# trinhvg/MoMA

Measured on AMD Instinct MI355X. Metric: images/sec MoMA train step (EffNet-B0 224px, K=65536), higher is better.
Workload: dtype bf16

## Files before the change

include/moma_hip.h:

```cpp
#ifndef MOMA_HIP_H
#define MOMA_HIP_H

#include <stddef.h>
#include <stdint.h>

#ifdef __cplusplus
extern "C" {
#endif

#define MOMA_ABI_VERSION 4

enum { MOMA_PREC_F32 = 0, MOMA_PREC_BF16 = 1 };
enum { MOMA_DT_F32 = 0, MOMA_DT_BF16 = 1 };

enum {
    MOMA_OK = 0,
    MOMA_E_NULL = -1,
    MOMA_E_SHAPE = -2,
    MOMA_E_DTYPE = -3,
    MOMA_E_ALIGN = -4,
    MOMA_E_WORKSPACE = -5,
    MOMA_E_UNSUPPORTED = -6
};

// ... 127 lines not shown
    const void* x;
    const void* pack;
    const float* b_qkv;
    const float* b_proj;
    float* y;
    void* qkv16;
    void* attn16;
    float* lse;
    void* qpack;
    float qpack_scale;
    int x_dtype;
} moma_mha_module_t;
size_t moma_mha_pack_bytes(int d);
int moma_mha_pack_weights(const float* w_qkv, const float* w_proj, void* pack, int d, int with_transposed,
                          moma_stream_t stream);
int moma_mha_fwd_fast(const moma_mha_module_t* modules, int n_modules, int N, int d, int H, moma_stream_t stream);
size_t moma_mha_bwd_fast_workspace_bytes(int N, int d, int H);
int moma_mha_bwd_fast(const void* pack, const void* x, int x_dtype, const void* qkv16, const void* attn16, const float* lse,
                      const float* dy, float* dx, float* dw_qkv, float* db_qkv, float* dw_proj, float* db_proj,
                      void* workspace, size_t workspace_bytes, int N, int d, int H, moma_stream_t stream);

enum { MOMA_ACT_NONE = 0, MOMA_ACT_SILU = 1, MOMA_ACT_RELU = 2 };
size_t moma_bn_workspace_bytes(int C);
int moma_bn_fwd(const void* x, void* out, const float* gamma, const float* beta, float* running_mean,
                float* running_var, float* save_mean, float* save_invstd, void* workspace,
                size_t workspace_bytes, int N, int C, int HW, int dtype, int act, int training,
                float momentum, float eps, void* plane_mean, moma_stream_t stream);
int moma_bn_bwd(const void* x, const void* dout, const float* gamma, const float* beta,
                const float* save_mean, const float* save_invstd, void* dx, float* dgamma, float* dbeta,
                void* workspace, size_t workspace_bytes, int N, int C, int HW, int dtype, int act,
                int training, const void* dplane_mean, moma_stream_t stream);
int moma_bn_prepare(const void* x, const float* gamma, const float* beta, float* running_mean,
                    float* running_var, float* save_mean, float* save_invstd, float* scale_shift,
                    void* workspace, size_t workspace_bytes, int N, int C, int HW, int dtype, int training,
                    float momentum, float eps, moma_stream_t stream);

size_t moma_dwconv_workspace_bytes(int C, int K);
int moma_dwconv_fwd(const void* x, const float* w, void* y, int N, int C, int H, int W, int OH, int OW,
                    int K, int stride, int pad_top, int pad_left, int dtype, moma_stream_t stream);
int moma_dwconv_bwd_data(const void* dy, const float* w, void* dx, int N, int C, int H, int W, int OH,
                         int OW, int K, int stride, int pad_top, int pad_left, int dtype,
                         moma_stream_t stream);
int moma_dwconv_bwd_weight(const void* x, const void* dy, float* dw, void* workspace,
                           size_t workspace_bytes, int N, int C, int H, int W, int OH, int OW, int K,
                           int stride, int pad_top, int pad_left, int dtype, moma_stream_t stream);
int moma_dwconv_fwd_pre(const void* x, const float* w, void* y, int N, int C, int H, int W, int OH, int OW,
                        int K, int stride, int pad_top, int pad_left, int dtype, const float* scale_shift,
                        int act, moma_stream_t stream);
int moma_dwconv_bwd_weight_pre(const void* x, const void* dy, float* dw, void* workspace,
                               size_t workspace_bytes, int N, int C, int H, int W, int OH, int OW, int K,
                               int stride, int pad_top, int pad_left, int dtype, const float* scale_shift,
                               int act, moma_stream_t stream);

int moma_plane_mean(const void* x, void* mean, int NC, int HW, int dtype, moma_stream_t stream);
int moma_se_gate_fwd(const void* x, const void* s, void* out, int NC, int HW, int dtype, moma_stream_t stream);
int moma_se_gate_bwd(const void* x, const void* s, const void* dout, void* dx, void* ds, int NC, int HW,
                     int dtype, moma_stream_t stream);

#ifdef __cplusplus
}
#endif
#endif
```

moma_amd/_lib.py:

```python
from __future__ import annotations

import ctypes as C
import os

_HERE = os.path.dirname(os.path.abspath(__file__))
LIB_PATH = os.environ.get("MOMA_HIP_LIB", os.path.join(_HERE, "lib", "libmoma_hip.so"))

PREC_F32, PREC_BF16 = 0, 1
DT_F32, DT_BF16 = 0, 1
LAYOUT_NCHW, LAYOUT_NHWC = 0, 1
NST_MAX_C, NST_ROW_BLOCK = 256, 32
RKD_MAX_B = 1024
SP_MAX_B = 1024
PKT_MAX_B = 1024
MHA_SAVE_PROBS, MHA_SAVE_LSE = 0, 1
ABI_VERSION = 4
EMA_BLOCK_ELEMS = 4096

_p = C.c_void_p
_i = C.c_int
_l = C.c_int64
_f = C.c_float
_z = C.c_size_t

# ... 6 lines not shown
    "moma_enqueue_mirror": (_i, [_p, _p, _p, _i, _l, _i, _i, _p]),
    "moma_queue_prefetch": (_i, [_p, _z, _p]),
    "moma_infonce_logits": (_i, [_p, _p, _p, _p, _i, _i, _i, _f, _i, _i, _p]),
    "moma_infonce_logits_bwd": (_i, [_p, _p, _p, _p, _i, _i, _i, _f, _i, _i, _p]),
    "moma_infonce_logits_bwd_workspace_bytes": (_z, [_i, _i, _i]),
    "moma_infonce_logits_bwd_ws": (_i, [_p, _p, _p, _p, _i, _i, _i, _f, _i, _i, _p, _z, _p]),
    "moma_infonce_logits_bwd_kq": (_i, [_p, _p, _p, _p, _i, _i, _i, _f, _i, _p]),
    "moma_infonce_fused_workspace_bytes": (_z, [_i, _i, _i, _i, _i]),
    "moma_infonce_fused": (_i, [_p, _p, _p, _i, _i, _i, _f, _p, _p, _p, _p, _p, _z, _i, _i, _p]),
    "moma_infonce_fused_ex": (_i, [_p, _p, _p, _i, _i, _i, _f, _p, _p, _p, _p, _p, _z, _i, _i, _p, _p, _p]),
    "moma_infonce_qpack_bytes": (_z, [_i, _i]),
    "moma_infonce_fused_q": (_i, [_p, _p, _p, _p, _i, _i, _i, _f, _p, _p, _p, _p, _p, _z, _i, _i, _p, _p, _p, _p]),
    "moma_infonce_fused_enqueue": (_i, [_p, _p, _p, _p, _i, _i, _i, _f, _p, _p, _p, _p, _p, _z, _i, _i, _p, _i, _l, _p, _p, _p, _p, _p]),
    "moma_infonce_fused_multi_workspace_bytes": (_z, [_i, _i, _i, _i, _i, _i]),
    "moma_infonce_fused_multi": (_i, [_p, _i, _i, _i, _i, _f, _p, _z, _i, _i, _p]),
    "moma_crd_workspace_bytes": (_z, [_i, _i, _i]),
    "moma_crd_fused": (_i, [_p, _p, _p, _p, _p, _i, _i, _i, _l, _f, _p, _i, _p, _p, _p, _p, _p, _z, _p]),
    "moma_crd_scores": (_i, [_p, _p, _p, _p, _p, _i, _i, _i, _l, _f, _p, _i, _p, _p, _p, _p, _z, _p]),
    "moma_crd_scores_bwd": (_i, [_p, _p, _p, _p, _p, _p, _p, _i, _i, _i, _l, _f, _p, _p, _p, _p, _z, _p]),
    "moma_crd_update": (_i, [_p, _p, _p, _p, _p, _i, _i, _l, _f, _p, _p]),
    "moma_at_workspace_bytes": (_z, [_i] * 8),
    "moma_at_map": (_i, [_p, _p] + [_i] * 8 + [_p, _z, _p]),
    "moma_at_pair": (_i, [_p, _p, _i, _i, _p, _p, _p, _p, _p, _p, _p, _p]),
    "moma_at_bwd": (_i, [_p, _p, _p, _p] + [_i] * 8 + [_p]),
    "moma_nst_workspace_bytes": (_z, [_i] * 3),
    "moma_nst_gram": (_i, [_p, _p] + [_i] * 8 + [_p, _z, _p, _p, _p, _p, _p, _p]),
    "moma_nst_bwd": (_i, [_p, _p, _p, _z, _p, _p, _p, _p] + [_i] * 8 + [_p]),
    "moma_rkd_workspace_bytes": (_z, [_i]),
    "moma_rkd_dist": (_i, [_p, _i, _i, _i, _p, _p]),
    "moma_rkd_terms": (_i, [_p, _p, _i, _f, _f, _p, _z, _p, _p, _p, _p]),
    "moma_rkd_bwd": (_i, [_p, _p, _p, _p, _i, _i, _i, _p]),
    "moma_sp_workspace_bytes": (_z, [_i, _l]),
    "moma_sp_gram": (_i, [_p, _i, _l, _i, _p, _z, _p]),
    "moma_sp_terms": (_i, [_p, _z, _l, _p, _z, _l, _i, _p, _p, _p, _p, _p, _p]),
    "moma_sp_bwd": (_i, [_p, _p, _p, _p, _i, _l, _i, _p]),
    "moma_pkt_workspace_bytes": (_z, [_i]),
    "moma_pkt_gram": (_i, [_p, _i, _i, _i, _p, _p]),
    "moma_pkt_gram_pair": (_i, [_p, _i, _i, _p, _i, _i, _i, _p, _p, _p]),
    "moma_pkt_terms":(_i, [_p, _p, _i, _p, _z, _p, _p, _p]),
    "moma_pkt_bwd": (_i, [_p, _p, _p, _p, _i, _i, _i, _p]),
    "moma_mha_fwd": (_i,[_p, _p, _p, _p, _p, _p, _p, _p, _p, _i, _i, _i, _i, _p]),
    "moma_mha_saved_state": (_i, [_i, _i, _i, _i]),
    "moma_mha_pack_bytes": (_z, [_i]),
    "moma_mha_pack_weights": (_i, [_p, _p, _p, _i, _i, _p]),
    "moma_mha_fwd_fast": (_i, [_p, _i, _i, _i, _i, _p]),
    "moma_mha_bwd_fast_workspace_bytes": (_z, [_i, _i, _i]),
    "moma_mha_bwd_fast": (_i, [_p, _p, _i, _p, _p, _p, _p, _p, _p, _p, _p, _p, _p, _z, _i, _i, _i, _p]),
    "moma_dwconv_workspace_bytes": (_z, [_i, _i]),
    "moma_dwconv_fwd": (_i, [_p, _p, _p] + [_i] * 11 + [_p]),
    "moma_dwconv_bwd_data": (_i, [_p, _p, _p] + [_i] * 11 + [_p]),
    "moma_dwconv_bwd_weight": (_i, [_p, _p, _p, _p, _z] + [_i] * 11 + [_p]),
    "moma_dwconv_fwd_pre": (_i, [_p, _p, _p] + [_i] * 11 + [_p, _i, _p]),
    "moma_dwconv_bwd_weight_pre": (_i, [_p, _p, _p, _p, _z] + [_i] * 11 + [_p, _i, _p]),
    "moma_plane_mean": (_i, [_p, _p, _i, _i, _i, _p]),
    "moma_se_gate_fwd": (_i, [_p, _p, _p, _i, _i, _i, _p]),
    "moma_se_gate_bwd": (_i, [_p, _p, _p, _p, _p, _i, _i, _i, _p]),
    "moma_bn_workspace_bytes": (_z, [_i]),
    "moma_bn_fwd": (_i, [_p, _p, _p, _p, _p, _p, _p, _p, _p, _z, _i, _i, _i, _i, _i, _i, _f, _f, _p, _p]),
    "moma_bn_bwd": (_i, [_p, _p, _p, _p, _p, _p, _p, _p, _p, _p, _z, _i, _i, _i, _i, _i, _i, _p, _p]),
    "moma_bn_prepare": (_i, [_p, _p, _p, _p, _p, _p, _p, _p, _p, _z, _i, _i, _i, _i, _i, _f, _f, _p]),
    "moma_mha_bwd_workspace_bytes": (_z, [_i, _i, _i, _i]),
    "moma_mha_bwd": (_i, [_p, _p, _p, _p, _p, _p, _p, _p, _p, _p, _p, _p, _p, _z, _i, _i, _i, _i, _p]),
}



class InfoNCETerm(C.Structure):
    _fields_ = [("q", _p), ("k", _p), ("queue", _p), ("loss_rows", _p), ("lse", _p), ("top1", _p), ("dq", _p)]


class MhaModule(C.Structure):
    _fields_ = [("x", _p), ("pack", _p), ("b_qkv", _p), ("b_proj", _p), ("y", _p), ("qkv16", _p), ("attn16", _p),
                ("lse", _p), ("qpack", _p), ("qpack_scale", _f), ("x_dtype", _i)]


_lib = None


class MomaHipError(RuntimeError):
    pass


def load():
    global _lib
    if _lib is not None:
        return _lib
    import torch
    if not os.path.exists(LIB_PATH):
        raise MomaHipError(
            f"libmoma_hip.so not found at {LIB_PATH}: build it with `python -m moma_amd.build` "
            "(hipcc --offload-arch=gfx950). There is no CPU fallback for the MoMA hot path.")
    lib = C.CDLL(LIB_PATH)
    for name, (res, args) in SIGNATURES.items():
        try:
            fn = getattr(lib, name)
        except AttributeError as e:
            raise MomaHipError(f"{LIB_PATH} does not export {name}") from e
        fn.restype = res
        fn.argtypes = args
    v = lib.moma_version()
    if v != ABI_VERSION:
        raise MomaHipError(f"libmoma_hip ABI version {v} != binding version {ABI_VERSION}; rebuild")
    _lib = lib
    return lib


# ... 5 lines not shown
```

moma_amd/backbones/efficientnet.py:

```python
import math
import os

import torch
import torch.nn as nn
import torch.nn.functional as F

_DW_MODE = os.environ.get("MOMA_DW", "hip")
_BN_MODE = os.environ.get("MOMA_BN", "hip")
_SE_MODE = os.environ.get("MOMA_SE", "hip")
_BNDW_FUSE = os.environ.get("MOMA_BNDW", "1")

_B0_STAGES = [
    (1, 3, 1, 1, 32, 16, 0.25),
    (2, 3, 2, 6, 16, 24, 0.25),
    (2, 5, 2, 6, 24, 40, 0.25),
    (3, 3, 2, 6, 40, 80, 0.25),
    (3, 5, 1, 6, 80, 112, 0.25),
    (4, 5, 2, 6, 112, 192, 0.25),
    (1, 3, 1, 6, 192, 320, 0.25),
]
_BN_MOM, _BN_EPS = 0.01, 1e-3


class _DepthwiseNative(torch.autograd.Function):

    @staticmethod
    def forward(ctx, x, w, stride, padding, groups):
        w = w.to(x.dtype)
        with torch.backends.cudnn.flags(enabled=False):
            y = F.conv2d(x, w, None, stride, padding, 1, groups)
        ctx.save_for_backward(x, w)
        ctx.cfg = (stride, padding, groups)
        return y

    @staticmethod
    def backward(ctx, gy):
        x, w = ctx.saved_tensors
        stride, padding, groups = ctx.cfg
        pad = padding if isinstance(padding, (tuple, list)) else (padding, padding)
        with torch.backends.cudnn.flags(enabled=False):
            gx, gw, _ = torch.ops.aten.convolution_backward(
                gy.contiguous(), x, w, None, list(stride), list(pad), [1, 1], False, [0, 0], groups,
                [ctx.needs_input_grad[0], ctx.needs_input_grad[1], False])
        return gx, (gw.float() if gw is not None else None), None, None, None


class _CachedCast(torch.autograd.Function):

    @staticmethod
    def forward(ctx, master, cached):
        ctx.dtype = master.dtype
        return cached.view_as(cached)

    @staticmethod
    def backward(ctx, g):
        return g.to(ctx.dtype), None


_WCACHE = os.environ.get("MOMA_WCACHE", "1") == "1"


def _same_pad(ih, iw, kh, kw, sh, sw):
    return (max((math.ceil(ih / sh) - 1) * sh + kh - ih, 0), max((math.ceil(iw / sw) - 1) * sw + kw - iw, 0))


class SamePadConv2d(nn.Conv2d):

    def __init__(self, cin, cout, kernel_size, stride=1, groups=1, bias=True):
        super().__init__(cin, cout, kernel_size, stride=stride, padding=0, groups=groups, bias=bias)
        self._wc = self._bc = None
        self._wc_live = False

    def _params(self, x):
        if self._wc_live and x.is_cuda and x.dtype == torch.bfloat16:
            track = torch.is_grad_enabled()
            w = _CachedCast.apply(self.weight, self._wc) if (track and self.weight.requires_grad) else self._wc
            b = None
            if self.bias is not None:
                b = _CachedCast.apply(self.bias, self._bc) if (track and self.bias.requires_grad) else self._bc
            return w, b
        return self.weight, self.bias

    def _is_depthwise(self):
        return self.groups > 1 and self.groups == self.in_channels == self.out_channels and self.bias is None

    def forward(self, x):
        ih, iw = x.shape[-2:]
        kh, kw = self.kernel_size
        sh, sw = self.stride
        ph, pw = _same_pad(ih, iw, kh, kw, sh, sw)
        depthwise = self._is_depthwise()
        if depthwise and x.is_cuda and _DW_MODE == "hip" and kh == kw and sh == sw and self.dilation == (1, 1):
            from .. import ops
            if ops.dwconv_supported(kh, sh):
                if torch.is_autocast_enabled():
                    x = x.to(torch.get_autocast_dtype("cuda"))
                if x.dtype in (torch.float32, torch.bfloat16):
                    return ops.dwconv(x, self.weight, sh, ph // 2, pw // 2, math.ceil(ih / sh), math.ceil(iw / sw))
        pad = (ph // 2, pw // 2)
        if ph % 2 or pw % 2:
            x = F.pad(x, [pw // 2, pw - pw // 2, ph // 2, ph - ph // 2])
            pad = 0
        if depthwise and x.is_cuda and _DW_MODE in ("hip", "aten"):
            if torch.is_autocast_enabled():
                x = x.to(torch.get_autocast_dtype("cuda"))
            return _DepthwiseNative.apply(x, self.weight, self.stride, pad, self.groups)
        if self._wc_live and torch.is_autocast_enabled() and x.is_cuda and x.dtype != torch.bfloat16 and \
                torch.get_autocast_dtype("cuda") == torch.bfloat16:
            x = x.to(torch.bfloat16)
        w, b = self._params(x)
        return F.conv2d(x, w, b, self.stride, pad, self.dilation, self.groups)


class BatchNorm2d(nn.BatchNorm2d):

    _nbt_pending = 0

    def _flush_nbt(self):
        if self._nbt_pending and self.num_batches_tracked is not None:
            self.num_batches_tracked.add_(self._nbt_pending)
        self._nbt_pending = 0

    def _save_to_state_dict(self, destination, prefix, keep_vars):
        self._flush_nbt()
        super()._save_to_state_dict(destination, prefix, keep_vars)

    def _load_from_state_dict(self, *args, **kwargs):
        self._nbt_pending = 0
        super()._load_from_state_dict(*args, **kwargs)

    def forward(self, x, act=None, want_mean=False):
        if _BN_MODE == "hip" and x.is_cuda and x.dtype in (torch.float32, torch.bfloat16) and self.momentum is not None:
            from .. import ops
            use_batch = self.training or self.running_mean is None
            if self.training and self.track_running_stats and self.num_batches_tracked is not None:
                self._nbt_pending += 1
            return ops.bn_act(x, self.weight, self.bias, self.running_mean, self.running_var, use_batch,
                              self.momentum, self.eps, act, want_mean)
        if _BN_MODE == "aten" and x.is_cuda:
            with torch.backends.cudnn.flags(enabled=False):
                y = super().forward(x)
        else:
            y = super().forward(x)
        y = F.silu(y) if act == "silu" else (F.relu(y) if act == "relu" else y)
        return (y, F.adaptive_avg_pool2d(y, 1)) if want_mean else y


def _drop_connect(x, p, training):
    if not training or not p:
        return x
    keep = 1.0 - p
    mask = torch.floor(keep + torch.rand([x.shape[0], 1, 1, 1], dtype=x.dtype, device=x.device))
    return x / keep * mask


class MBConvBlock(nn.Module):
    def __init__(self, kernel, stride, expand, cin, cout, se_ratio):
        super().__init__()
        mid = cin * expand
        self.expand, self.stride, self.cin, self.cout = expand, stride, cin, cout
        if expand != 1:
            self._expand_conv = SamePadConv2d(cin, mid, 1, bias=False)
            self._bn0 = BatchNorm2d(mid, momentum=_BN_MOM, eps=_BN_EPS)
# ... 134 lines not shown
```

moma_amd/csrc/api.hip:

```cpp
#include "common.hpp"

using namespace moma;

namespace {
inline int hip_rc(hipError_t e) { return e == hipSuccess ? MOMA_OK : (int)e; }
inline bool bad_prec(int p) { return p != MOMA_PREC_F32 && p != MOMA_PREC_BF16; }
inline bool bad_dt(int t) { return t != MOMA_DT_F32 && t != MOMA_DT_BF16; }
inline bool misaligned(const void* p, size_t a) { return ((uintptr_t)p % a) != 0; }
inline size_t align_up(size_t x, size_t a) { return (x + a - 1) / a * a; }

#define MOMA_TRY(expr)                         \
    do {                                       \
        hipError_t _e = (expr);                \
        if (_e != hipSuccess) return (int)_e;  \
    } while (0)

GemmArgs gemm(const float* A, const void* B, float* C, int M, int N, int K, long lda, long ldb, long ldc, int tA,
              int tB, float alpha, int prec) {
    GemmArgs g{};
    g.A = A; g.B = B; g.C = C; g.bias = nullptr;
    g.M = M; g.N = N; g.K = K; g.lda = lda; g.ldb = ldb; g.ldc = ldc;
    g.strideA = g.strideB = g.strideC = 0; g.batch = 1;
    g.transA = tA; g.transB = tB; g.alpha = alpha; g.splitk = 1; g.atomic = 0; g.splitC = 0;
    g.b_dtype = MOMA_DT_F32; g.prec = prec;
// ... 471 lines not shown

int moma_dwconv_fwd(const void* x, const float* w, void* y, int N, int C, int H, int W, int OH, int OW, int K, int stride,
                    int pad_top, int pad_left, int dtype, moma_stream_t stream) {
    if (!x || !w || !y) return MOMA_E_NULL;
    const int rc = dw_check(N, C, H, W, OH, OW, K, stride, pad_top, pad_left, dtype);
    if (rc != MOMA_OK) return rc;
    return hip_rc(launch_dw_fwd(x, w, y, N, C, H, W, OH, OW, K, stride, pad_top, pad_left, dtype, nullptr, MOMA_ACT_NONE,
                                (hipStream_t)stream));
}

static bool bad_act(int act) { return act != MOMA_ACT_NONE && act != MOMA_ACT_SILU && act != MOMA_ACT_RELU; }

int moma_dwconv_fwd_pre(const void* x, const float* w, void* y, int N, int C, int H, int W, int OH, int OW, int K, int stride,
                        int pad_top, int pad_left, int dtype, const float* scale_shift, int act, moma_stream_t stream) {
    if (!x || !w || !y || !scale_shift) return MOMA_E_NULL;
    const int rc = dw_check(N, C, H, W, OH, OW, K, stride, pad_top, pad_left, dtype);
    if (rc != MOMA_OK) return rc;
    if (bad_act(act)) return MOMA_E_DTYPE;
    return hip_rc(launch_dw_fwd(x, w, y, N, C, H, W, OH, OW, K, stride, pad_top, pad_left, dtype, scale_shift, act,
                                (hipStream_t)stream));
}

int moma_dwconv_bwd_data(const void* dy, const float* w, void* dx, int N, int C, int H, int W, int OH, int OW, int K,
                         int stride, int pad_top, int pad_left, int dtype, moma_stream_t stream) {
    if (!dy || !w || !dx) return MOMA_E_NULL;
    const int rc = dw_check(N, C, H, W, OH, OW, K, stride, pad_top, pad_left, dtype);
    if (rc != MOMA_OK) return rc;
    return hip_rc(launch_dw_bwd_data(dy, w, dx, N, C, H, W, OH, OW, K, stride, pad_top, pad_left, dtype, (hipStream_t)stream));
}

int moma_dwconv_bwd_weight(const void* x, const void* dy, float* dw, void* workspace, size_t workspace_bytes, int N, int C,
                           int H, int W, int OH, int OW, int K, int stride, int pad_top, int pad_left, int dtype,
                           moma_stream_t stream) {
    if (!x || !dy || !dw || !workspace) return MOMA_E_NULL;
    const int rc = dw_check(N, C, H, W, OH, OW, K, stride, pad_top, pad_left, dtype);
    if (rc != MOMA_OK) return rc;
    if (workspace_bytes < moma_dwconv_workspace_bytes(C, K)) return MOMA_E_WORKSPACE;
    return hip_rc(launch_dw_bwd_weight(x, dy, dw, (float*)workspace, workspace_bytes / sizeof(float), N, C, H, W, OH, OW, K,
                                       stride, pad_top, pad_left, dtype, nullptr, MOMA_ACT_NONE, (hipStream_t)stream));
}

int moma_dwconv_bwd_weight_pre(const void* x, const void* dy, float* dw, void* workspace, size_t workspace_bytes, int N, int C,
                               int H, int W, int OH, int OW, int K, int stride, int pad_top, int pad_left, int dtype,
                               const float* scale_shift, int act, moma_stream_t stream) {
    if (!x || !dy || !dw || !workspace || !scale_shift) return MOMA_E_NULL;
    const int rc = dw_check(N, C, H, W, OH, OW, K, stride, pad_top, pad_left, dtype);
    if (rc != MOMA_OK) return rc;
    if (bad_act(act)) return MOMA_E_DTYPE;
    if (workspace_bytes < moma_dwconv_workspace_bytes(C, K)) return MOMA_E_WORKSPACE;
    return hip_rc(launch_dw_bwd_weight(x, dy, dw, (float*)workspace, workspace_bytes / sizeof(float), N, C, H, W, OH, OW, K,
                                       stride, pad_top, pad_left, dtype, scale_shift, act, (hipStream_t)stream));
}

static int se_check(int NC, int HW, int dtype) {
    if (NC <= 0 || HW <= 0) return MOMA_E_SHAPE;
    if (dtype != MOMA_DT_F32 && dtype != MOMA_DT_BF16) return MOMA_E_DTYPE;
    return MOMA_OK;
}
int moma_plane_mean(const void* x, void* mean, int NC, int HW, int dtype, moma_stream_t stream) {
    if (!x || !mean) return MOMA_E_NULL;
    const int rc = se_check(NC, HW, dtype);
    return rc != MOMA_OK ? rc : hip_rc(launch_plane_mean(x, mean, NC, HW, dtype, (hipStream_t)stream));
}
int moma_se_gate_fwd(const void* x, const void* s, void* out, int NC, int HW, int dtype, moma_stream_t stream) {
    if (!x || !s || !out) return MOMA_E_NULL;
    const int rc = se_check(NC, HW, dtype);
    return rc != MOMA_OK ? rc : hip_rc(launch_se_gate_fwd(x, s, out, NC, HW, dtype, (hipStream_t)stream));
}
int moma_se_gate_bwd(const void* x, const void* s, const void* dout, void* dx, void* ds, int NC, int HW, int dtype,
                     moma_stream_t stream) {
    if (!x || !s || !dout || !dx || !ds) return MOMA_E_NULL;
    const int rc = se_check(NC, HW, dtype);
    return rc != MOMA_OK ? rc : hip_rc(launch_se_gate_bwd(x, s, dout, dx, ds, NC, HW, dtype, (hipStream_t)stream));
}

static int crd_check(int B, int d, int K1, int64_t n_data, float T) {
    if (B <= 0 || d < 4 || d % 4 != 0 || K1 < 2 || n_data <= 0 || !(T > 0.f)) return MOMA_E_SHAPE;
    if (d > 2048 || B > 65535) return MOMA_E_UNSUPPORTED;
    return MOMA_OK;
}
static bool crd_misaligned(const void* a, const void* b, const void* c, const void* d, const void* e = nullptr,
                           const void* f = nullptr, const void* g = nullptr, const void* h = nullptr) {
    return misaligned(a, 16) || misaligned(b, 16) || misaligned(c, 16) || misaligned(d, 16) || misaligned(e, 16) ||
           misaligned(f, 16) || misaligned(g, 16) || misaligned(h, 16);
}

size_t moma_crd_workspace_bytes(int B, int d, int K1) {
    if (crd_check(B, d, K1, 1, 1.f) != MOMA_OK) return 0;
    return crd_workspace_bytes(B, d, K1);
}

int moma_crd_fused(const float* v1, const float* v2, const float* memory_v1, const float* memory_v2, const int64_t* idx,
                   int B, int d, int K1, int64_t n_data, float T, float* Z, int set_z, float* loss, float* dv1, float* dv2,
                   int32_t* bad_index, void* workspace, size_t workspace_bytes, moma_stream_t stream) {
    if (!v1 || !v2 || !memory_v1 || !memory_v2 || !idx || !Z || !loss || !bad_index || !workspace) return MOMA_E_NULL;
    if ((dv1 == nullptr) != (dv2 == nullptr)) return MOMA_E_NULL;
    const int rc = crd_check(B, d, K1, n_data, T);
    if (rc != MOMA_OK) return rc;
    if (crd_misaligned(v1, v2, memory_v1, memory_v2, dv1, dv2, workspace) || misaligned(idx, 8) || misaligned(Z, 4) ||
        misaligned(loss, 4) || misaligned(bad_index, 4))
        return MOMA_E_ALIGN;
    if (workspace_bytes < crd_workspace_bytes(B, d, K1)) return MOMA_E_WORKSPACE;
    return hip_rc(launch_crd_fused(v1, v2, memory_v1, memory_v2, idx, B, d, K1, n_data, T, Z, set_z, loss, dv1, dv2, bad_index,
                                   workspace, (hipStream_t)stream));
}

// ... 272 lines not shown
```

moma_amd/csrc/common.hpp:

```cpp
#pragma once
#include <hip/hip_runtime.h>
#include <stdint.h>
#include <initializer_list>
#include <type_traits>
#include "../../include/moma_hip.h"

namespace moma {

typedef __attribute__((ext_vector_type(8))) __bf16 bf16x8;
typedef __attribute__((ext_vector_type(4))) __bf16 bf16x4;
typedef __attribute__((ext_vector_type(4))) float f32x4;
typedef __attribute__((ext_vector_type(16))) float f32x16;
typedef unsigned short bf16_raw;

constexpr int WAVE = 64;

__device__ __forceinline__ float bf16_to_f32(bf16_raw v) {
    return __uint_as_float(((unsigned)v) << 16);
}
__device__ __forceinline__ bf16_raw f32_to_bf16(float f) {
    __bf16 b = (__bf16)f;
    return *reinterpret_cast<bf16_raw*>(&b);
}

// ... 242 lines not shown
    void* queue16;
    float* queue32;
    const float* rows;
    int n;
    int64_t index;
    int K, d;
};
hipError_t launch_infonce_flash(const float* q, const float* k, const void* queue, int B, int d, int K, float inv_T,
                                float* loss_rows, float* lse, int32_t* top1, float* dq, void* ws, int qdtype,
                                hipStream_t st, hipEvent_t ev_begin = nullptr, hipEvent_t ev_end = nullptr,
                                const void* q_packed = nullptr, hipEvent_t ev_call_end = nullptr,
                                const EnqueueJob* enq = nullptr);
size_t infonce_qpack_bytes(int B, int d);
bool infonce_multi_supported(int n_terms, int B, int d, int K, int qdtype, int prec);
size_t infonce_multi_workspace_bytes(int n_terms, int B, int d, int K);
hipError_t launch_infonce_multi(const moma_infonce_term_t* terms, int n_terms, int B, int d, int K, float inv_T, void* ws,
                                hipStream_t st);

bool infonce_f32_flash_supported(int B, int d, int K, int qdtype, int prec);
size_t infonce_f32_flash_workspace_bytes(int B, int d, int K);
hipError_t launch_infonce_f32_flash(const float* q, const float* k, const float* queue, int B, int d, int K, float inv_T,
                                    float* loss_rows, float* lse, int32_t* top1, float* dq, void* ws, hipStream_t st,
                                    hipEvent_t ev_begin = nullptr, hipEvent_t ev_end = nullptr);

bool mha_fast_supported(int N, int d, int H, int prec);
hipError_t launch_mha_pack(const float* w_qkv, const float* w_proj, void* pack, int d, int with_t, hipStream_t st);
hipError_t launch_mha_fwd_fast(const moma_mha_module_t* mods, int n_modules, int N, int d, int H, hipStream_t st);
size_t mha_bwd_fast_workspace_bytes(int N, int d);
hipError_t launch_mha_bwd_fast(const void* pack, const void* x, int x_dtype, const void* qkv16, const void* attn16, const float* lse,
                               const float* dy, float* dx, float* dw_qkv, float* db_qkv, float* dw_proj, float* db_proj,
                               void* workspace, int N, int d, int H, hipStream_t st);

size_t bn_workspace_floats(int C);
hipError_t launch_bn_fwd(const void* x, void* out, const float* gamma, const float* beta, float* rm, float* rv,
                         float* save_mean, float* save_invstd, float* ws, int N, int C, int HW, int dtype, int act,
                         int training, float momentum, float eps, void* plane_mean, hipStream_t st);
hipError_t launch_bn_prepare(const void* x, const float* gamma, const float* beta, float* rm, float* rv, float* save_mean,
                             float* save_invstd, float* scale_shift, float* ws, int N, int C, int HW, int dtype, int training,
                             float momentum, float eps, hipStream_t st);
hipError_t launch_bn_bwd(const void* x, const void* dout, const float* gamma, const float* beta, const float* save_mean,
                         const float* save_invstd, void* dx, float* dgamma, float* dbeta, float* ws, int N, int C, int HW,
                         int dtype, int act, int training, const void* dplane_mean, hipStream_t st);

bool dwconv_supported(int K, int S);
size_t dwconv_workspace_floats(int C, int K);
hipError_t launch_dw_fwd(const void* x, const float* w, void* y, int N, int C, int H, int W, int OH, int OW, int K, int S,
                         int pt, int pl, int dtype, const float* scale_shift, int act, hipStream_t st);
hipError_t launch_dw_bwd_data(const void* dy, const float* w, void* dx, int N, int C, int H, int W, int OH, int OW, int K,
                              int S, int pt, int pl, int dtype, hipStream_t st);
hipError_t launch_dw_bwd_weight(const void* x, const void* dy, float* dw, float* ws, size_t ws_floats, int N, int C, int H,
                                int W, int OH, int OW, int K, int S, int pt, int pl, int dtype, const float* scale_shift, int act,
                                hipStream_t st);

hipError_t launch_plane_mean(const void* x, void* out, int NC, int HW, int dtype, hipStream_t st);
hipError_t launch_se_gate_fwd(const void* x, const void* s, void* out, int NC, int HW, int dtype, hipStream_t st);
hipError_t launch_se_gate_bwd(const void* x, const void* s, const void* dout, void* dx, void* ds, int NC, int HW, int dtype,
                              hipStream_t st);

}
```

moma_amd/ops.py:

```python
from __future__ import annotations

import ctypes as C
from typing import Sequence, Tuple

import torch

from . import _lib
from ._lib import DT_BF16, DT_F32, PREC_BF16, PREC_F32, EMA_BLOCK_ELEMS, MomaHipError, check

_PREC = {"fp32": PREC_F32, "f32": PREC_F32, "float32": PREC_F32, PREC_F32: PREC_F32,
         "bf16": PREC_BF16, "bfloat16": PREC_BF16, PREC_BF16: PREC_BF16}


def prec_code(p) -> int:
    try:
        return _PREC[p]
    except KeyError:
        raise ValueError(f"unknown precision {p!r}; use 'fp32' or 'bf16'")


def _qdtype(queue: torch.Tensor) -> int:
    if queue.dtype == torch.float32:
        return DT_F32
    if queue.dtype == torch.bfloat16:
# ... 608 lines not shown
    return _BNAct.apply(x, weight, bias, running_mean, running_var, bool(training), momentum, eps, ACT_CODES[act],
                        bool(want_mean))


class _DWConv(torch.autograd.Function):
    @staticmethod
    def forward(ctx, x, w, stride, pad_top, pad_left, out_h, out_w):
        lib = _lib.load()
        _dev(x, "x", dtype=None, contiguous=False)
        _dev(w, "weight")
        if x.dim() != 4 or x.dtype not in _DT_CODES or w.dim() != 4 or w.shape[1] != 1 or w.shape[0] != x.shape[1] \
                or w.shape[2] != w.shape[3]:
            raise ValueError(f"dwconv: x {tuple(x.shape)} {x.dtype}, weight {tuple(w.shape)}")
        x = x.contiguous()
        w = w.contiguous()
        N, Cc, H, W = x.shape
        K = w.shape[2]
        y = torch.empty(N, Cc, out_h, out_w, device=x.device, dtype=x.dtype)
        check(lib.moma_dwconv_fwd(_ptr(x), _ptr(w), _ptr(y), N, Cc, H, W, out_h, out_w, K, stride, pad_top, pad_left,
                                  _DT_CODES[x.dtype], _stream()), "moma_dwconv_fwd")
        ctx.save_for_backward(x, w)
        ctx.cfg = (N, Cc, H, W, out_h, out_w, K, stride, pad_top, pad_left)
        return y

    @staticmethod
    def backward(ctx, dy):
        lib = _lib.load()
        x, w = ctx.saved_tensors
        N, Cc, H, W, OH, OW, K, stride, pt, pl = ctx.cfg
        dy = dy.contiguous()
        if dy.dtype != x.dtype:
            dy = dy.to(x.dtype)
        dx = dw = None
        if ctx.needs_input_grad[0]:
            dx = torch.empty_like(x)
            check(lib.moma_dwconv_bwd_data(_ptr(dy), _ptr(w), _ptr(dx), N, Cc, H, W, OH, OW, K, stride, pt, pl,
                                           _DT_CODES[x.dtype], _stream()), "moma_dwconv_bwd_data")
        if ctx.needs_input_grad[1]:
            dw = torch.empty_like(w)
            ws = torch.empty(lib.moma_dwconv_workspace_bytes(Cc, K), device=x.device, dtype=torch.uint8)
            check(lib.moma_dwconv_bwd_weight(_ptr(x), _ptr(dy), _ptr(dw), _ptr(ws), ws.numel(), N, Cc, H, W, OH, OW, K,
                                             stride, pt, pl, _DT_CODES[x.dtype], _stream()), "moma_dwconv_bwd_weight")
        return dx, dw, None, None, None, None, None


def dwconv_supported(kernel: int, stride: int) -> bool:
    return kernel in (3, 5) and stride in (1, 2)


def dwconv(x, weight, stride: int, pad_top: int, pad_left: int, out_h: int, out_w: int):
    return _DWConv.apply(x, weight, int(stride), int(pad_top), int(pad_left), int(out_h), int(out_w))


class _BNActDWConv(torch.autograd.Function):
    @staticmethod
    def forward(ctx, x, weight, bias, running_mean, running_var, training, momentum, eps, act, w, stride, pad_top,
                pad_left, out_h, out_w):
        lib = _lib.load()
        _dev(x, "x", dtype=None, contiguous=False)
        _dev(w, "weight")
        if x.dim() != 4 or x.dtype not in _DT_CODES or w.dim() != 4 or w.shape[1] != 1 or w.shape[0] != x.shape[1] \
                or w.shape[2] != w.shape[3]:
            raise ValueError(f"bn_act_dwconv: x {tuple(x.shape)} {x.dtype}, weight {tuple(w.shape)}")
        x = x.contiguous()
        w = w.contiguous()
        N, Cc, H, W = x.shape
        K = w.shape[2]
        dev = x.device
        save_mean = torch.empty(Cc, device=dev, dtype=torch.float32)
        save_invstd = torch.empty(Cc, device=dev, dtype=torch.float32)
        scale_shift = torch.empty(Cc, 2, device=dev, dtype=torch.float32)
        ws = torch.empty(lib.moma_bn_workspace_bytes(Cc), device=dev, dtype=torch.uint8)
        check(lib.moma_bn_prepare(_ptr(x), _ptr(weight), _ptr(bias), _ptr(running_mean), _ptr(running_var), _ptr(save_mean),
                                  _ptr(save_invstd), _ptr(scale_shift), _ptr(ws), ws.numel(), N, Cc, H * W,
                                  _DT_CODES[x.dtype], int(training), float(momentum), float(eps), _stream()), "moma_bn_prepare")
        y = torch.empty(N, Cc, out_h, out_w, device=dev, dtype=x.dtype)
        check(lib.moma_dwconv_fwd_pre(_ptr(x), _ptr(w), _ptr(y), N, Cc, H, W, out_h, out_w, K, stride, pad_top, pad_left,
                                      _DT_CODES[x.dtype], _ptr(scale_shift), act, _stream()), "moma_dwconv_fwd_pre")
        ctx.save_for_backward(x, weight, bias, save_mean, save_invstd, scale_shift, w)
        ctx.cfg = (N, Cc, H, W, out_h, out_w, K, stride, pad_top, pad_left, act, int(training))
        ctx.set_materialize_grads(False)
        return y

    @staticmethod
    def backward(ctx, dy):
        lib = _lib.load()
        x, weight, bias, save_mean, save_invstd, scale_shift, w = ctx.saved_tensors
        N, Cc, H, W, OH, OW, K, stride, pt, pl, act, training = ctx.cfg
        dx = dgamma = dbeta = dw = None
        if dy is None:
            return (None,) * 15
        dy = dy.contiguous()
        if dy.dtype != x.dtype:
            dy = dy.to(x.dtype)
        dev, dt = x.device, _DT_CODES[x.dtype]
        want_gamma = weight is not None and ctx.needs_input_grad[1]
        want_beta = bias is not None and ctx.needs_input_grad[2]
        if ctx.needs_input_grad[0] or want_gamma or want_beta:
            da = torch.empty_like(x)
            check(lib.moma_dwconv_bwd_data(_ptr(dy), _ptr(w), _ptr(da), N, Cc, H, W, OH, OW, K, stride, pt, pl, dt,
                                           _stream()), "moma_dwconv_bwd_data")
            dx = torch.empty_like(x) if ctx.needs_input_grad[0] else None
            dgamma = torch.empty(Cc, device=dev, dtype=torch.float32) if want_gamma else None
            dbeta = torch.empty(Cc, device=dev, dtype=torch.float32) if want_beta else None
            ws = torch.empty(lib.moma_bn_workspace_bytes(Cc), device=dev, dtype=torch.uint8)
            check(lib.moma_bn_bwd(_ptr(x), _ptr(da), _ptr(weight), _ptr(bias), _ptr(save_mean), _ptr(save_invstd), _ptr(dx),
# ... 557 lines not shown
```

Baseline: 6505.

## Add split-K MFMA kernel for pointwise conv weight gradient

Adds a custom HIP kernel that computes the 1x1 conv weight gradient as a bf16 MFMA GEMM over the pixel dimension. It splits the reduction across many workgroups, writes fp32 partials to a workspace and sums them in a finalize kernel. EfficientNet pointwise convs are routed through a new autograd function that uses this kernel for dW and keeps aten for dx. The intent is to replace the library weight-gradient path, which is inefficient for small-channel, large-spatial shapes. The cost is extra workspace traffic and a second kernel launch per conv.

```diff
diff --git a/include/moma_hip.h b/include/moma_hip.h
--- a/include/moma_hip.h
+++ b/include/moma_hip.h
@@ -203,6 +203,10 @@
                                int stride, int pad_top, int pad_left, int dtype, const float* scale_shift,
                                int act, moma_stream_t stream);
 
+size_t moma_pwconv_workspace_bytes(int N, int Cin, int Cout, int HW);
+int moma_pwconv_bwd_weight(const void* x, const void* dy, void* dw, void* workspace, size_t workspace_bytes, int N, int Cin,
+                           int Cout, int HW, int dtype, moma_stream_t stream);
+
 int moma_plane_mean(const void* x, void* mean, int NC, int HW, int dtype, moma_stream_t stream);
 int moma_se_gate_fwd(const void* x, const void* s, void* out, int NC, int HW, int dtype, moma_stream_t stream);
 int moma_se_gate_bwd(const void* x, const void* s, const void* dout, void* dx, void* ds, int NC, int HW,
diff --git a/moma_amd/_lib.py b/moma_amd/_lib.py
--- a/moma_amd/_lib.py
+++ b/moma_amd/_lib.py
@@ -82,6 +82,8 @@
     "moma_dwconv_bwd_weight": (_i, [_p, _p, _p, _p, _z] + [_i] * 11 + [_p]),
     "moma_dwconv_fwd_pre": (_i, [_p, _p, _p] + [_i] * 11 + [_p, _i, _p]),
     "moma_dwconv_bwd_weight_pre": (_i, [_p, _p, _p, _p, _z] + [_i] * 11 + [_p, _i, _p]),
+    "moma_pwconv_workspace_bytes": (_z, [_i, _i, _i, _i]),
+    "moma_pwconv_bwd_weight": (_i, [_p, _p, _p, _p, _z] + [_i] * 5 + [_p]),
     "moma_plane_mean": (_i, [_p, _p, _i, _i, _i, _p]),
     "moma_se_gate_fwd": (_i, [_p, _p, _p, _i, _i, _i, _p]),
     "moma_se_gate_bwd": (_i, [_p, _p, _p, _p, _p, _i, _i, _i, _p]),
diff --git a/moma_amd/backbones/efficientnet.py b/moma_amd/backbones/efficientnet.py
--- a/moma_amd/backbones/efficientnet.py
+++ b/moma_amd/backbones/efficientnet.py
@@ -9,6 +9,7 @@
 _BN_MODE = os.environ.get("MOMA_BN", "hip")
 _SE_MODE = os.environ.get("MOMA_SE", "hip")
 _BNDW_FUSE = os.environ.get("MOMA_BNDW", "1")
+_PW_MODE = os.environ.get("MOMA_PW", "hip")
 
 _B0_STAGES = [
     (1, 3, 1, 1, 32, 16, 0.25),
@@ -83,6 +84,13 @@
 
     def _is_depthwise(self):
         return self.groups > 1 and self.groups == self.in_channels == self.out_channels and self.bias is None
+
+    def _is_pointwise(self):
+        return (self.kernel_size == (1, 1) and self.stride == (1, 1) and self.dilation == (1, 1) and self.groups == 1
+                and self.padding == (0, 0))
+
+    def _takes_pwconv(self, is_cuda, dtype):
+        return _PW_MODE == "hip" and self._wc_live and is_cuda and dtype == torch.bfloat16 and self._is_pointwise()
 
     def forward(self, x):
         ih, iw = x.shape[-2:]
@@ -109,6 +117,9 @@
                 torch.get_autocast_dtype("cuda") == torch.bfloat16:
             x = x.to(torch.bfloat16)
         w, b = self._params(x)
+        if self._takes_pwconv(x.is_cuda, x.dtype) and torch.is_grad_enabled() and w.requires_grad:
+            from .. import ops
+            return ops.pwconv(x, w, b)
         return F.conv2d(x, w, b, self.stride, pad, self.dilation, self.groups)
 
 
diff --git a/moma_amd/csrc/api.hip b/moma_amd/csrc/api.hip
--- a/moma_amd/csrc/api.hip
+++ b/moma_amd/csrc/api.hip
@@ -547,6 +547,24 @@
                                        stride, pad_top, pad_left, dtype, scale_shift, act, (hipStream_t)stream));
 }
 
+static bool pw_bad_shape(int N, int Cin, int Cout, int HW) {
+    return N <= 0 || Cin <= 0 || Cout <= 0 || HW <= 0 || Cin > 65536 || Cout > 65536 || (long)N * HW > 0x7fffffffL;
+}
+
+size_t moma_pwconv_workspace_bytes(int N, int Cin, int Cout, int HW) {
+    return pw_bad_shape(N, Cin, Cout, HW) ? 0 : align_up(pwconv_workspace_floats(N, Cin, Cout, HW) * sizeof(float), 256);
+}
+
+int moma_pwconv_bwd_weight(const void* x, const void* dy, void* dw, void* workspace, size_t workspace_bytes, int N, int Cin,
+                           int Cout, int HW, int dtype, moma_stream_t stream) {
+    if (!x || !dy || !dw || !workspace) return MOMA_E_NULL;
+    if (pw_bad_shape(N, Cin, Cout, HW)) return MOMA_E_SHAPE;
+    if (dtype != MOMA_DT_BF16) return MOMA_E_DTYPE;
+    if (misaligned(x, 2) || misaligned(dy, 2) || misaligned(dw, 2) || misaligned(workspace, 16)) return MOMA_E_ALIGN;
+    if (workspace_bytes < moma_pwconv_workspace_bytes(N, Cin, Cout, HW)) return MOMA_E_WORKSPACE;
+    return hip_rc(launch_pw_bwd_weight(x, dy, dw, (float*)workspace, N, Cin, Cout, HW, (hipStream_t)stream));
+}
+
 static int se_check(int NC, int HW, int dtype) {
     if (NC <= 0 || HW <= 0) return MOMA_E_SHAPE;
     if (dtype != MOMA_DT_F32 && dtype != MOMA_DT_BF16) return MOMA_E_DTYPE;
diff --git a/moma_amd/csrc/common.hpp b/moma_amd/csrc/common.hpp
--- a/moma_amd/csrc/common.hpp
+++ b/moma_amd/csrc/common.hpp
@@ -318,6 +318,10 @@
                                 int W, int OH, int OW, int K, int S, int pt, int pl, int dtype, const float* scale_shift, int act,
                                 hipStream_t st);
 
+size_t pwconv_workspace_floats(int N, int Cin, int Cout, int HW);
+hipError_t launch_pw_bwd_weight(const void* x, const void* dy, void* dw, float* ws, int N, int Cin, int Cout, int HW,
+                                hipStream_t st);
+
 hipError_t launch_plane_mean(const void* x, void* out, int NC, int HW, int dtype, hipStream_t st);
 hipError_t launch_se_gate_fwd(const void* x, const void* s, void* out, int NC, int HW, int dtype, hipStream_t st);
 hipError_t launch_se_gate_bwd(const void* x, const void* s, const void* dout, void* dx, void* ds, int NC, int HW, int dtype,
diff --git a/moma_amd/csrc/pwconv.hip b/moma_amd/csrc/pwconv.hip
--- /dev/null
+++ b/moma_amd/csrc/pwconv.hip
@@ -0,0 +1,249 @@
+#include "common.hpp"
+
+namespace moma {
+namespace {
+
+constexpr int PW_WAVES = 4;
+constexpr int PW_UNIT = 64;
+constexpr int PW_TARGET_WAVES = 4096;
+constexpr int PW_MAX_SPLITS = 2048;
+
+struct PwPlan {
+    int tm, tn;
+    int mt, nt;
+    int imgs, hwk;
+    int cpp;
+    long units;
+    int splits;
+};
+
+int pw_tiles_per_wave(int tiles) { return tiles >= 3 ? 4 : tiles; }
+
+PwPlan pw_plan(int N, int Cin, int Cout, int HW) {
+    PwPlan p{};
+    const int tiles_m = (Cout + 15) / 16, tiles_n = (Cin + 15) / 16;
+    p.tm = pw_tiles_per_wave(tiles_m);
+    p.tn = pw_tiles_per_wave(tiles_n);
+    p.mt = (tiles_m + p.tm - 1) / p.tm;
+    p.nt = (tiles_n + p.tn - 1) / p.tn;
+    p.imgs = HW == 1 ? 1 : N;
+    p.hwk = HW == 1 ? N : HW;
+    p.cpp = (p.hwk + PW_UNIT - 1) / PW_UNIT;
+    p.units = (long)p.imgs * p.cpp;
+    const long wave_tiles = (long)p.mt * p.nt;
+    const long in_bytes = (long)N * HW * ((long)Cin + Cout) * 2, out_bytes = (long)Cout * Cin * 4;
+    long s = (PW_TARGET_WAVES + wave_tiles - 1) / wave_tiles;
+    if (s > in_bytes / (2 * out_bytes)) s = in_bytes / (2 * out_bytes);
+    if (s > p.units) s = p.units;
+    if (s > PW_MAX_SPLITS) s = PW_MAX_SPLITS;
+    if (s < 1) s = 1;
+    p.splits = (int)s;
+    return p;
+}
+
+struct PwArgs {
+    const bf16_raw* x;
+    const bf16_raw* dy;
+    float* part;
+    int Cin, Cout, hwk, cpp, mt, nt, splits;
+    long units;
+    long x_img, dy_img;
+    long x_row, dy_row;
+    long x_pix, dy_pix;
+};
+
+template <int VEC>
+__device__ __forceinline__ void pw_load16(const bf16_raw* __restrict__ row, long pix, int pl, int hwk, unsigned (&w)[8]) {
+    if constexpr (VEC == 8) {
+#pragma unroll
+        for (int g = 0; g < 2; ++g) {
+            const uint4 v = *reinterpret_cast<const uint4*>(row + (pl + 8 * g < hwk ? pl + 8 * g : 0));
+            w[4 * g] = v.x; w[4 * g + 1] = v.y; w[4 * g + 2] = v.z; w[4 * g + 3] = v.w;
+        }
+    } else if constexpr (VEC == 4) {
+#pragma unroll
+        for (int g = 0; g < 4; ++g) {
+            const uint2 v = *reinterpret_cast<const uint2*>(row + (pl + 4 * g < hwk ? pl + 4 * g : 0));
+            w[2 * g] = v.x; w[2 * g + 1] = v.y;
+        }
+    } else {
+        unsigned e[16];
+#pragma unroll
+        for (int i = 0; i < 16; ++i) {
+            const bool ok = pl + i < hwk;
+            const unsigned v = row[ok ? (long)(pl + i) * pix : 0];
+            e[i] = ok ? v : 0u;
+        }
+#pragma unroll
+        for (int i = 0; i < 8; ++i) w[i] = e[2 * i] | (e[2 * i + 1] << 16);
+    }
+}
+template <int VEC>
+__device__ __forceinline__ void pw_mask16(int pl, int hwk, unsigned (&w)[8]) {
+    if constexpr (VEC > 1) {
+#pragma unroll
+        for (int i = 0; i < 8; ++i) w[i] = pl + (2 * i / VEC) * VEC < hwk ? w[i] : 0u;
+    }
+}
+
+__device__ __forceinline__ bf16x8 pw_frag(const unsigned* w) {
+    typedef unsigned u4 __attribute__((ext_vector_type(4)));
+    const u4 v = {w[0], w[1], w[2], w[3]};
+    return __builtin_bit_cast(bf16x8, v);
+}
+
+template <int TM, int TN, int VEC>
+__global__ __launch_bounds__(PW_WAVES * 64) void pw_wgrad_kernel(PwArgs a) {
+    const int lane = threadIdx.x & 63, wave = threadIdx.x >> 6;
+    const int r = lane & 15, q = lane >> 4;
+    const int wt = blockIdx.x * PW_WAVES + wave;
+    if (wt >= a.mt * a.nt) return;
+    const int wm = wt / a.nt, wn = wt - wm * a.nt;
+    const int s = blockIdx.y;
+    const long u0 = a.units * s / a.splits, u1 = a.units * (s + 1) / a.splits;
+
+    long aoff[TM], boff[TN];
+#pragma unroll
+    for (int i = 0; i < TM; ++i) aoff[i] = (long)min((wm * TM + i) * 16 + r, a.Cout - 1) * a.dy_row;
+#pragma unroll
+    for (int j = 0; j < TN; ++j) boff[j] = (long)min((wn * TN + j) * 16 + r, a.Cin - 1) * a.x_row;
+
+    f32x4 acc[TM][TN];
+#pragma unroll
+    for (int i = 0; i < TM; ++i)
+#pragma unroll
+        for (int j = 0; j < TN; ++j) acc[i][j] = f32x4{0.f, 0.f, 0.f, 0.f};
+
+    int n = (int)(u0 / a.cpp), c = (int)(u0 - (long)n * a.cpp);
+    unsigned af0[TM][8], bf0[TN][8], af1[TM][8], bf1[TN][8];
+    int pl0 = 0, pl1 = 0;
+    auto load = [&](unsigned (&af)[TM][8], unsigned (&bf)[TN][8], int& pl) {
+        pl = c * PW_UNIT + 16 * q;
+        const bf16_raw* ap = a.dy + (long)n * a.dy_img;
+        const bf16_raw* bp = a.x + (long)n * a.x_img;
+#pragma unroll
+        for (int i = 0; i < TM; ++i) pw_load16<VEC>(ap + aoff[i], a.dy_pix, pl, a.hwk, af[i]);
+#pragma unroll
+        for (int j = 0; j < TN; ++j) pw_load16<VEC>(bp + boff[j], a.x_pix, pl, a.hwk, bf[j]);
+        if (++c == a.cpp) { c = 0; ++n; }
+    };
+    auto mma = [&](unsigned (&af)[TM][8], unsigned (&bf)[TN][8], int pl) {
+        if (pl + 16 > a.hwk) {
+#pragma unroll
+            for (int i = 0; i < TM; ++i) pw_mask16<VEC>(pl, a.hwk, af[i]);
+#pragma unroll
+            for (int j = 0; j < TN; ++j) pw_mask16<VEC>(pl, a.hwk, bf[j]);
+        }
+#pragma unroll
+        for (int h = 0; h < 2; ++h)
+#pragma unroll
+            for (int i = 0; i < TM; ++i)
+#pragma unroll
+                for (int j = 0; j < TN; ++j)
+                    acc[i][j] = __builtin_amdgcn_mfma_f32_16x16x32_bf16(pw_frag(af[i] + 4 * h), pw_frag(bf[j] + 4 * h), acc[i][j],
+                                                                        0, 0, 0);
+    };
+    long u = u0;
+    if (u < u1) load(af0, bf0, pl0);
+    while (u < u1) {
+        const bool more0 = u + 1 < u1;
+        if (more0) load(af1, bf1, pl1);
+        mma(af0, bf0, pl0);
+        if (!more0) break;
+        ++u;
+        const bool more1 = u + 1 < u1;
+        if (more1) load(af0, bf0, pl0);
+        mma(af1, bf1, pl1);
+        if (!more1) break;
+        ++u;
+    }
+
+    float* part = a.part + (size_t)s * a.Cout * a.Cin;
+#pragma unroll
+    for (int i = 0; i < TM; ++i)
+#pragma unroll
+        for (int j = 0; j < TN; ++j) {
+            const int ci = (wn * TN + j) * 16 + r;
+#pragma unroll
+            for (int v = 0; v < 4; ++v) {
+                const int co = (wm * TM + i) * 16 + 4 * q + v;
+                if (co < a.Cout && ci < a.Cin) part[(size_t)co * a.Cin + ci] = acc[i][j][v];
+            }
+        }
+}
+
+template <int G>
+__global__ __launch_bounds__(G == 1 ? 256 : 16 * G) void pw_finalize_kernel(const float* __restrict__ part,
+                                                                           bf16_raw* __restrict__ dw, long total, int splits) {
+    constexpr int E = G == 1 ? 256 : 16;
+    const int el = threadIdx.x % E, g = threadIdx.x / E;
+    const long e = (long)blockIdx.x * E + el;
+    const long ec = e < total ? e : total - 1;
+    float sum = 0.f;
+    for (int s0 = g; s0 < splits; s0 += 8 * G) {
+        float v[8];
+#pragma unroll
+        for (int i = 0; i < 8; ++i) v[i] = part[(size_t)min(s0 + i * G, splits - 1) * total + ec];
+#pragma unroll
+        for (int i = 0; i < 8; ++i) sum += s0 + i * G < splits ? v[i] : 0.f;
+    }
+    if constexpr (G > 1) {
+        __shared__ float sm[G][E];
+        sm[g][el] = sum;
+        __syncthreads();
+        if (g != 0) return;
+        sum = sm[0][el];
+#pragma unroll
+        for (int k = 1; k < G; ++k) sum += sm[k][el];
+    }
+    if (e < total) dw[e] = f32_to_bf16(sum);
+}
+
+template <int TM, int TN>
+void pw_launch_tile(const PwArgs& a, int vec, dim3 grid, hipStream_t st) {
+    with_vec<8, 8, 4, 1>(vec, [&](auto V) {
+        hipLaunchKernelGGL((pw_wgrad_kernel<TM, TN, V>), grid, dim3(PW_WAVES * 64), 0, st, a);
+    });
+}
+
+}
+
+size_t pwconv_workspace_floats(int N, int Cin, int Cout, int HW) {
+    return (size_t)pw_plan(N, Cin, Cout, HW).splits * Cout * Cin;
+}
+
+hipError_t launch_pw_bwd_weight(const void* x, const void* dy, void* dw, float* ws, int N, int Cin, int Cout, int HW,
+                                hipStream_t st) {
+    const PwPlan p = pw_plan(N, Cin, Cout, HW);
+    PwArgs a{};
+    a.x = (const bf16_raw*)x; a.dy = (const bf16_raw*)dy; a.part = ws;
+    a.Cin = Cin; a.Cout = Cout; a.hwk = p.hwk; a.cpp = p.cpp; a.mt = p.mt; a.nt = p.nt; a.splits = p.splits; a.units = p.units;
+    int vec = 1;
+    if (HW == 1) {
+        a.x_img = a.dy_img = 0; a.x_row = a.dy_row = 1; a.x_pix = Cin; a.dy_pix = Cout;
+    } else {
+        a.x_img = (long)Cin * HW; a.dy_img = (long)Cout * HW; a.x_row = a.dy_row = HW; a.x_pix = a.dy_pix = 1;
+        vec = pick_vec(HW, 2, (uintptr_t)x | (uintptr_t)dy, {8, 4});
+    }
+    const dim3 grid((unsigned)(((long)p.mt * p.nt + PW_WAVES - 1) / PW_WAVES), (unsigned)p.splits);
+#define MOMA_PW_ROW(TMV)                                             \
+    if (p.tn == 1) pw_launch_tile<TMV, 1>(a, vec, grid, st);         \
+    else if (p.tn == 2) pw_launch_tile<TMV, 2>(a, vec, grid, st);    \
+    else pw_launch_tile<TMV, 4>(a, vec, grid, st);
+    if (p.tm == 1) { MOMA_PW_ROW(1) }
+    else if (p.tm == 2) { MOMA_PW_ROW(2) }
+    else { MOMA_PW_ROW(4) }
+#undef MOMA_PW_ROW
+    hipError_t e = hipGetLastError();
+    if (e != hipSuccess) return e;
+    const long total = (long)Cout * Cin;
+    if (p.splits > 32)
+        hipLaunchKernelGGL(pw_finalize_kernel<64>, dim3((unsigned)((total + 15) / 16)), dim3(1024), 0, st, ws, (bf16_raw*)dw, total,
+                           p.splits);
+    else
+        hipLaunchKernelGGL(pw_finalize_kernel<1>, dim3((unsigned)((total + 255) / 256)), dim3(256), 0, st, ws, (bf16_raw*)dw, total,
+                           p.splits);
+    return hipGetLastError();
+}
+
+}
diff --git a/moma_amd/ops.py b/moma_amd/ops.py
--- a/moma_amd/ops.py
+++ b/moma_amd/ops.py
@@ -684,6 +684,61 @@
     return _DWConv.apply(x, weight, int(stride), int(pad_top), int(pad_left), int(out_h), int(out_w))
 
 
+def pwconv_native(N: int, Cin: int, Cout: int, HW: int) -> bool:
+    return HW == 1 or HW % 4 == 0
+
+
+def pwconv_bwd_weight(x, dy):
+    lib = _lib.load()
+    _dev(x, "x", dtype=torch.bfloat16, contiguous=False)
+    _dev(dy, "dy", dtype=torch.bfloat16, contiguous=False)
+    if x.dim() != 4 or dy.dim() != 4 or x.shape[0] != dy.shape[0] or x.shape[2:] != dy.shape[2:]:
+        raise ValueError(f"pwconv_bwd_weight: x {tuple(x.shape)}, dy {tuple(dy.shape)}")
+    x = x.contiguous()
+    dy = dy.contiguous()
+    N, Cin, H, W = x.shape
+    Cout = dy.shape[1]
+    dw = torch.empty(Cout, Cin, 1, 1, device=x.device, dtype=torch.bfloat16)
+    ws = torch.empty(lib.moma_pwconv_workspace_bytes(N, Cin, Cout, H * W), device=x.device, dtype=torch.uint8)
+    check(lib.moma_pwconv_bwd_weight(_ptr(x), _ptr(dy), _ptr(dw), _ptr(ws), ws.numel(), N, Cin, Cout, H * W, DT_BF16, _stream()),
+          "moma_pwconv_bwd_weight")
+    return dw
+
+
+class _PWConv(torch.autograd.Function):
+    @staticmethod
+    def forward(ctx, x, w, b):
+        _dev(x, "x", dtype=torch.bfloat16, contiguous=False)
+        _dev(w, "weight", dtype=torch.bfloat16, contiguous=False)
+        if x.dim() != 4 or w.dim() != 4 or w.shape[1] != x.shape[1] or w.shape[2:] != (1, 1):
+            raise ValueError(f"pwconv: x {tuple(x.shape)}, weight {tuple(w.shape)}")
+        ctx.save_for_backward(x, w)
+        ctx.has_bias = b is not None
+        return torch.nn.functional.conv2d(x, w, b)
+
+    @staticmethod
+    def backward(ctx, dy):
+        x, w = ctx.saved_tensors
+        dx = dw = db = None
+        if ctx.needs_input_grad[0]:
+            dx = torch.ops.aten.convolution_backward(dy, x, w, None, [1, 1], [0, 0], [1, 1], False, [0, 0], 1,
+                                                     [True, False, False])[0]
+        if ctx.needs_input_grad[1]:
+            N, Cin, H, W = x.shape
+            if pwconv_native(N, Cin, w.shape[0], H * W):
+                dw = pwconv_bwd_weight(x, dy)
+            else:
+                dw = torch.ops.aten.convolution_backward(dy, x, w, None, [1, 1], [0, 0], [1, 1], False, [0, 0], 1,
+                                                         [False, True, False])[1]
+        if ctx.has_bias and ctx.needs_input_grad[2]:
+            db = dy.sum((0, 2, 3))
+        return dx, dw, db
+
+
+def pwconv(x, w, b=None):
+    return _PWConv.apply(x, w, b)
+
+
 class _BNActDWConv(torch.autograd.Function):
     @staticmethod
     def forward(ctx, x, weight, bias, running_mean, running_var, training, momentum, eps, act, w, stride, pad_top,
```

New measurement: 6791 (median of 6 runs). 4.4% higher.
